# PaddlePaddle/MetaGym

Hardware: AMD Instinct MI355X
Metric: env-steps/sec (whole node) at 2^16 parallel envs; 1/2/4/8-GPU scaling (higher is better)
Workload: dtype f32/f64 mixed (reference choreography)

## Files before the change

### include/metagym_hip.h

```cpp
#ifndef METAGYM_HIP_H
#define METAGYM_HIP_H

#include <stddef.h>
#include <stdint.h>

#ifdef __cplusplus
extern "C" {
#endif

#define MG_ABI_VERSION 10

#define MG_OK 0
#define MG_ERR_NULL_POINTER (-1001)
#define MG_ERR_BAD_SIZE (-1002)
#define MG_ERR_BAD_CONFIG (-1003)
#define MG_ERR_UNSUPPORTED (-1004)

int mg_abi_version(void);
const char *mg_last_error(void);
const char *mg_target_arch(void);

int mg_selftest_philox(const uint32_t *ctr_key_d, uint32_t *out_d, int32_t n, void *stream);


// ... 63 lines not shown
                                const mg_quadrotor_state *state, const mg_quadrotor_autoreset *ar,
                                const float *action, float *obs, float *reward, double *reward64,
                                uint8_t *done, uint8_t *failed, void *stream);

typedef struct mg_quadrotor_plan { uint64_t opaque[128]; } mg_quadrotor_plan;

int mg_quadrotor_plan_init(mg_quadrotor_plan *plan, const mg_quadrotor_config *cfg,
                           const mg_quadrotor_autoreset *ar , int32_t n_envs,
                           const mg_quadrotor_state *state);
int mg_quadrotor_plan_step(const mg_quadrotor_plan *plan, int32_t n_steps, const float *action, float *obs,
                           float *reward, double *reward64, uint8_t *done, uint8_t *failed, void *stream);

typedef struct mg_quadrotor_fold {
    int32_t one_wave_form;
    uint32_t span;
    uint32_t base_v, base_w;
    uint32_t edge_v, edge_w;
    float pos_safe32;
    float fail_range_sq32;
    double fail_velocity, fail_w;
} mg_quadrotor_fold;

int mg_quadrotor_plan_fold(const mg_quadrotor_plan *plan, mg_quadrotor_fold *out);

typedef struct mg_quadrotor_tasks {
    const void *rows_d;
    const int32_t *task_id_d;
    const float *velocity_targets_d;
    int32_t n_tasks;
    int32_t all_simple;
    double dt;
} mg_quadrotor_tasks;

typedef struct mg_quadrotor_task_fold {
    float inertia_inv[9];
    float lm[4];
    float fail_range_sq32;
    float prec32;
    int32_t times;
    int32_t simple;
    double precision, half_dt2, dt;
    float init_velocity[3], init_angular_velocity[3];
    double init_velocity_noisy, init_angular_velocity_noisy;
} mg_quadrotor_task_fold;

int32_t mg_quadrotor_tasks_row_bytes(void);
// ... 599 lines not shown
```

### metagym_amd/_lib.py

```python
import ctypes as C
import os

from . import build as _build

ABI_VERSION = 10

MG_OK = 0


class MetaGymHipError(RuntimeError):
    pass


class QuadrotorConfig(C.Structure):
    _fields_ = [
        ("precision", C.c_double), ("quality", C.c_double),
        ("ct0", C.c_double), ("ct1", C.c_double), ("ct2", C.c_double),
        ("mm", C.c_double), ("jm", C.c_double), ("ra", C.c_double), ("phi", C.c_double),
        ("fail_velocity", C.c_double), ("fail_w", C.c_double), ("fail_range", C.c_double),
        ("min_voltage", C.c_double), ("max_voltage", C.c_double),
        ("dt", C.c_double), ("healthy_reward", C.c_double), ("z_offset", C.c_double),
        ("x_offset", C.c_int64), ("y_offset", C.c_int64),
        ("nt", C.c_int32), ("task", C.c_int32),
        ("inertia", C.c_float * 9), ("drag_m", C.c_float * 9), ("drag_f", C.c_float * 9),
# ... 267 lines not shown
                  "pyp", "pyv", "npp", "npv", "reward", "timec", "energy", "given", "st_d", "st_g", "st_a", "st_e", "st_w",
                  "rp_holder", "rp_priority"]
LIFTSIM_POLICY_ACTIONS, LIFTSIM_POLICY_RULE = 0, 1

_P = C.c_void_p
SIGNATURES = {
    "mg_abi_version": (C.c_int, []),
    "mg_last_error": (C.c_char_p, []),
    "mg_target_arch": (C.c_char_p, []),
    "mg_selftest_philox": (C.c_int, [_P, _P, C.c_int32, _P]),
    "mg_quadrotor_default_config": (C.c_int, [C.POINTER(QuadrotorConfig)]),
    "mg_quadrotor_velocity_targets": (C.c_int, [C.POINTER(QuadrotorConfig), C.c_int32, _P, _P, _P]),
    "mg_quadrotor_reset": (C.c_int, [C.POINTER(QuadrotorConfig), C.c_int32, C.POINTER(QuadrotorState),
                                     _P, _P, _P, _P, _P]),
    "mg_quadrotor_step": (C.c_int, [C.POINTER(QuadrotorConfig), C.c_int32, C.POINTER(QuadrotorState),
                                    _P, _P, _P, _P, _P, _P, _P]),
    "mg_quadrotor_step_autoreset": (C.c_int, [C.POINTER(QuadrotorConfig), C.c_int32, C.c_int32,
                                              C.POINTER(QuadrotorState), C.POINTER(QuadrotorAutoReset),
                                              _P, _P, _P, _P, _P, _P, _P]),
    "mg_quadrotor_plan_init": (C.c_int, [C.POINTER(QuadrotorPlan), C.POINTER(QuadrotorConfig),
                                         C.POINTER(QuadrotorAutoReset), C.c_int32, C.POINTER(QuadrotorState)]),
    "mg_quadrotor_plan_step": (C.c_int, [C.POINTER(QuadrotorPlan), C.c_int32, _P, _P, _P, _P, _P, _P, _P]),
    "mg_quadrotor_plan_fold": (C.c_int, [C.POINTER(QuadrotorPlan), C.POINTER(QuadrotorFold)]),
    "mg_quadrotor_tasks_row_bytes": (C.c_int32, []),
    "mg_quadrotor_tasks_fold": (C.c_int, [C.POINTER(QuadrotorConfig), C.POINTER(QuadrotorAutoReset), _P]),
    "mg_quadrotor_tasks_describe": (C.c_int, [_P, C.POINTER(QuadrotorTaskFold)]),
    "mg_quadrotor_tasks_step": (C.c_int, [C.POINTER(QuadrotorConfig), C.POINTER(QuadrotorTasks), C.c_int32, C.c_int32,
                                          C.POINTER(QuadrotorState), C.POINTER(QuadrotorAutoReset),
                                          _P, _P, _P, _P, _P, _P, _P]),
    "mg_quadrotor_tasks_reset": (C.c_int, [C.POINTER(QuadrotorConfig), C.POINTER(QuadrotorTasks), C.c_int32,
                                           C.POINTER(QuadrotorState), _P, _P, _P, _P, _P]),
    "mg_quadrotor_policy_param_count": (C.c_int32, [C.c_int32, C.c_int32]),
    "mg_quadrotor_policy_rollout": (C.c_int, [C.POINTER(QuadrotorConfig), C.POINTER(QuadrotorTasks), C.c_int32, C.c_int32,
                                              C.POINTER(QuadrotorState), C.POINTER(QuadrotorAutoReset),
                                              C.POINTER(QuadrotorPolicyDesc), _P, _P, _P, C.POINTER(QuadrotorPolicyRecords),
                                              C.POINTER(QuadrotorPolicyLast), _P]),
    "mg_quadrotor_rpolicy_param_count": (C.c_int32, [C.c_int32, C.c_int32]),
    "mg_quadrotor_rpolicy_rollout": (C.c_int, [C.POINTER(QuadrotorConfig), C.POINTER(QuadrotorTasks), C.c_int32, C.c_int32,
                                               C.POINTER(QuadrotorState), C.POINTER(QuadrotorAutoReset),
                                               C.POINTER(QuadrotorPolicyDesc), C.POINTER(QuadrotorRPolicyCarry), C.c_int32,
                                               _P, _P, _P, C.POINTER(QuadrotorPolicyRecords),
                                               C.POINTER(QuadrotorPolicyLast), _P]),
    "mg_quadrotor_rollout": (C.c_int, [C.POINTER(QuadrotorConfig), C.c_int32, C.c_int32,
                                       C.POINTER(QuadrotorState), _P, _P, _P, _P, _P, _P, _P]),
    "mg_maze_view_tables": (C.c_int, [C.c_int32, C.c_double, C.c_double, _P, _P]),
    "mg_maze_sample_tasks": (C.c_int, [C.POINTER(MazeSampleParams), C.c_int32, C.c_uint32, _P, _P, _P, _P, _P, _P,
# ... 132 lines not shown
```

### metagym_amd/csrc/quadrotor.hip

```cpp
#include <cstdlib>
#include <cstring>

#include "mg_common.h"
#include "mg_philox.h"

namespace {

#ifndef MG_QUAD_BLOCK
#define MG_QUAD_BLOCK 256
#endif
constexpr int BLOCK = MG_QUAD_BLOCK;
constexpr int WAVES_PER_BLOCK = BLOCK / mg::WAVE;
constexpr int OBS_DIM = 16;

struct QuadK {
    float phi32, phi_over_ra32, inv_jm32, mm32, prec32, ct0_32, ct1_32;
    float quality32, dt32, zoff32, healthy32, fail_range_sq32;
    float lm[4];
    float pc[12];
    float iinv[9];
    float df[9], dm[9];
    float cog[3];
    double prec, half_dt2, half_dt, ct2, quality, inv_quality;
    double min_v, max_v, fail_velocity, fail_w, healthy, xoff, yoff;
// ... 425 lines not shown
constexpr int AUX_PLAIN = 0, AUX_NT = 2, AUX_SC1 = 16, AUX_SC0_SC1 = 17, AUX_SC1_NT = 18;
constexpr bool st_policy_ok(int aux) {
    return aux == AUX_PLAIN || aux == AUX_NT || aux == AUX_SC1 || aux == AUX_SC0_SC1 || aux == AUX_SC1_NT;
}
constexpr bool ld_policy_ok(int aux) { return aux == AUX_PLAIN || aux == AUX_NT; }
#ifndef MG_QUAD_ST_STATE
#define MG_QUAD_ST_STATE 16
#endif
#ifndef MG_QUAD_ST_OBS
#define MG_QUAD_ST_OBS 16
#endif
#ifndef MG_QUAD_ST_SCALAR
#define MG_QUAD_ST_SCALAR 16
#endif
#ifndef MG_QUAD_STP_STATE
#define MG_QUAD_STP_STATE 2
#endif
#ifndef MG_QUAD_STP_OBS
#define MG_QUAD_STP_OBS 2
#endif
#ifndef MG_QUAD_STP_SCALAR
#define MG_QUAD_STP_SCALAR 2
#endif
#ifndef MG_QUAD_LD_STATE
#define MG_QUAD_LD_STATE 0
#endif
static_assert(st_policy_ok(MG_QUAD_ST_STATE) && st_policy_ok(MG_QUAD_ST_OBS) && st_policy_ok(MG_QUAD_ST_SCALAR) &&
              st_policy_ok(MG_QUAD_STP_STATE) && st_policy_ok(MG_QUAD_STP_OBS) && st_policy_ok(MG_QUAD_STP_SCALAR),
              "store policy: 0 plain, 2 nt, 16 sc1, 17 sc0 sc1, 18 sc1 nt");
static_assert(ld_policy_ok(MG_QUAD_LD_STATE), "load policy: 0 plain, 2 nt");
enum StoreClass { ST_STATE = 0, ST_OBS = 1, ST_SCALAR = 2 };
template <bool BUF, int CLS> constexpr int st_policy() {
    return CLS == ST_STATE ? (BUF ? MG_QUAD_ST_STATE : MG_QUAD_STP_STATE)
         : CLS == ST_OBS   ? (BUF ? MG_QUAD_ST_OBS : MG_QUAD_STP_OBS)
                           : (BUF ? MG_QUAD_ST_SCALAR : MG_QUAD_STP_SCALAR);
}
typedef float v4f __attribute__((ext_vector_type(4)));
typedef uint32_t v2u __attribute__((ext_vector_type(2)));
typedef uint32_t v4u __attribute__((ext_vector_type(4)));

__device__ __forceinline__ __amdgpu_buffer_rsrc_t rsrc_of(const void *base, uint32_t bytes) {
    return __builtin_amdgcn_make_buffer_rsrc(const_cast<void *>(base), (short)0, (int)bytes, 0x00020000);
}
template <typename T, int AUX = AUX_PLAIN> __device__ __forceinline__ T buf_ld(__amdgpu_buffer_rsrc_t r, uint32_t vo, uint32_t so) {
    static_assert(ld_policy_ok(AUX), "load policy");
    if constexpr (sizeof(T) == 4) return __builtin_bit_cast(T, __builtin_amdgcn_raw_buffer_load_b32(r, vo, so, AUX));
    else if constexpr (sizeof(T) == 8) return __builtin_bit_cast(T, __builtin_amdgcn_raw_buffer_load_b64(r, vo, so, AUX));
    else return __builtin_bit_cast(T, __builtin_amdgcn_raw_buffer_load_b128(r, vo, so, AUX));
}
template <int AUX, typename T> __device__ __forceinline__ void buf_st(T v, __amdgpu_buffer_rsrc_t r, uint32_t vo, uint32_t so) {
    static_assert(st_policy_ok(AUX), "store policy");
    if constexpr (sizeof(T) == 1) __builtin_amdgcn_raw_buffer_store_b8(__builtin_bit_cast(uint8_t, v), r, vo, so, AUX);
    else if constexpr (sizeof(T) == 4) __builtin_amdgcn_raw_buffer_store_b32(__builtin_bit_cast(uint32_t, v), r, vo, so, AUX);
    else if constexpr (sizeof(T) == 8) __builtin_amdgcn_raw_buffer_store_b64(__builtin_bit_cast(v2u, v), r, vo, so, AUX);
    else __builtin_amdgcn_raw_buffer_store_b128(__builtin_bit_cast(v4u, v), r, vo, so, AUX);
}
template <typename T> struct same_size_uint;
template <> struct same_size_uint<uint8_t> { typedef uint8_t type; };
// ... 3 lines not shown
template <> struct same_size_uint<double> { typedef uint64_t type; };
template <int AUX, typename T> __device__ __forceinline__ void st_stream(T *p, T v) {
    static_assert(st_policy_ok(AUX), "store policy");
    if constexpr (AUX == AUX_NT) __builtin_nontemporal_store(v, p);
    else if constexpr (AUX == AUX_PLAIN) *p = v;
    else if constexpr (AUX == AUX_SC1 && sizeof(T) <= 8) {
        typedef typename same_size_uint<T>::type U;
        __hip_atomic_store(reinterpret_cast<U *>(p), __builtin_bit_cast(U, v), __ATOMIC_RELAXED, __HIP_MEMORY_SCOPE_AGENT);
    } else {
        const uint64_t a = (uint64_t)p;
        const uint64_t base = ((uint64_t)(uint32_t)__builtin_amdgcn_readfirstlane((uint32_t)(a >> 32)) << 32) |
                              (uint64_t)(uint32_t)__builtin_amdgcn_readfirstlane((uint32_t)a);
        buf_st<AUX>(v, rsrc_of((const void *)base, mg::WAVE * OBS_DIM * 4), (uint32_t)(a - base), 0);
    }
}
template <bool BUF, int AUX = AUX_PLAIN, typename T> __device__ __forceinline__ T ld_soa(const T *a, int comps, int n, int c, int e) {
    if (!BUF) {
        if constexpr (AUX == AUX_NT) return __builtin_nontemporal_load(&a[(size_t)c * n + e]);
        else return a[(size_t)c * n + e];
    }
    return buf_ld<T, AUX>(rsrc_of(a, (uint32_t)comps * (uint32_t)n * sizeof(T)), (uint32_t)e * sizeof(T),
                          (uint32_t)c * (uint32_t)n * sizeof(T));
}
template <bool BUF, int CLS, typename T> __device__ __forceinline__ void st_soa(T *a, int comps, int n, int c, int e, T v) {
    if (!BUF) return st_stream<st_policy<false, CLS>()>(&a[(size_t)c * n + e], v);
    buf_st<st_policy<true, CLS>()>(v, rsrc_of(a, (uint32_t)comps * (uint32_t)n * sizeof(T)), (uint32_t)e * sizeof(T),
                                   (uint32_t)c * (uint32_t)n * sizeof(T));
}

template <bool ROT_FIRST = false, bool BUF = false>
__device__ __forceinline__ void load_state(const mg_quadrotor_state &st, int n, int e, Lane &s, int &ct) {
    if (ROT_FIRST) {
#pragma unroll
        for (int c = 0; c < 9; ++c) s.R[c] = ld_soa<BUF, MG_QUAD_LD_STATE>(st.rot, 9, n, c, e);
    }
    if (!ROT_FIRST) {
#pragma unroll
        for (int c = 0; c < 3; ++c) s.p[c] = ld_soa<BUF, MG_QUAD_LD_STATE>(st.pos, 3, n, c, e);
    }
#pragma unroll
    for (int c = 0; c < 3; ++c) s.v[c] = ld_soa<BUF, MG_QUAD_LD_STATE>(st.vel, 3, n, c, e);
#pragma unroll
    for (int c = 0; c < 3; ++c) s.w[c] = ld_soa<BUF, MG_QUAD_LD_STATE>(st.omega, 3, n, c, e);
    if (ROT_FIRST) {
#pragma unroll
        for (int c = 0; c < 3; ++c) s.p[c] = ld_soa<BUF, MG_QUAD_LD_STATE>(st.pos, 3, n, c, e);
    }
#pragma unroll
    for (int c = 0; c < 4; ++c) s.pw[c] = ld_soa<BUF, MG_QUAD_LD_STATE>(st.propw, 4, n, c, e);
    if (!ROT_FIRST) {
#pragma unroll
        for (int c = 0; c < 9; ++c) s.R[c] = ld_soa<BUF, MG_QUAD_LD_STATE>(st.rot, 9, n, c, e);
    }
    ct = ld_soa<BUF, MG_QUAD_LD_STATE>(st.ct, 1, n, 0, e);
}

__device__ __forceinline__ void derive_lane(Lane &s) {
    update_derived(s);
    s.power = 0.0f;
}

template <bool BUF = false>
__device__ __forceinline__ void load_lane(const mg_quadrotor_state &st, int n, int e, Lane &s, int &ct) {
    load_state<false, BUF>(st, n, e, s, ct);
    derive_lane(s);
}

template <bool BUF = false>
__device__ __forceinline__ void store_lane(const mg_quadrotor_state &st, int n, int e, const Lane &s, int ct) {
#pragma unroll
    for (int c = 0; c < 3; ++c) st_soa<BUF, ST_STATE>(st.pos, 3, n, c, e, s.p[c]);
#pragma unroll
    for (int c = 0; c < 3; ++c) st_soa<BUF, ST_STATE>(st.vel, 3, n, c, e, s.v[c]);
#pragma unroll
    for (int c = 0; c < 3; ++c) st_soa<BUF, ST_STATE>(st.omega, 3, n, c, e, s.w[c]);
#pragma unroll
    for (int c = 0; c < 4; ++c) st_soa<BUF, ST_STATE>(st.propw, 4, n, c, e, s.pw[c]);
#pragma unroll
    for (int c = 0; c < 9; ++c) st_soa<BUF, ST_STATE>(st.rot, 9, n, c, e, s.R[c]);
    st_soa<BUF, ST_STATE>(st.ct, 1, n, 0, e, ct);
}

template <bool BUF = false>
__device__ __forceinline__ void store_obs_wave(float *tile, const float *obs, float *out, int n, int e, int obs_dim) {
    if (!BUF && obs_dim != OBS_DIM) {
        if (e < n)
            for (int c = 0; c < obs_dim; ++c) out[(size_t)e * obs_dim + c] = obs[c];
        return;
    }
    const int lane = threadIdx.x & (mg::WAVE - 1);
    const int wave_base = e - lane;
    const bool full = (wave_base + mg::WAVE) <= n;
    if (full) {
#pragma unroll
        for (int c = 0; c < OBS_DIM; ++c) tile[lane * (OBS_DIM + 1) + c] = obs[c];
        __builtin_amdgcn_wave_barrier();
        float4 *dst = reinterpret_cast<float4 *>(out + (size_t)wave_base * OBS_DIM);
        const __amdgpu_buffer_rsrc_t r = rsrc_of(out, (uint32_t)n * (OBS_DIM * 4));
#pragma unroll
        for (int j = 0; j < 4; ++j) {
            const int q = j * mg::WAVE + lane;
            const int row = q >> 2, col = (q & 3) * 4;
            const float *src = &tile[row * (OBS_DIM + 1) + col];
            const v4f v{src[0], src[1], src[2], src[3]};
            if (BUF) buf_st<st_policy<true, ST_OBS>()>(v, r, (uint32_t)(wave_base * OBS_DIM + 4 * lane) * 4 + j * (mg::WAVE * 16), 0);
            else st_stream<st_policy<false, ST_OBS>()>(reinterpret_cast<v4f *>(dst + q), v);
        }
        __builtin_amdgcn_wave_barrier();
    } else if (e < n) {
        float4 *dst = reinterpret_cast<float4 *>(out + (size_t)e * OBS_DIM);
        const __amdgpu_buffer_rsrc_t r = rsrc_of(out, (uint32_t)n * (OBS_DIM * 4));
#pragma unroll
        for (int j = 0; j < 4; ++j) {
            const v4f v{obs[4 * j], obs[4 * j + 1], obs[4 * j + 2], obs[4 * j + 3]};
            if (BUF) buf_st<st_policy<true, ST_OBS>() & ~AUX_NT>(v, r, (uint32_t)e * (OBS_DIM * 4) + j * 16, 0);
            else if constexpr ((st_policy<false, ST_OBS>() & ~AUX_NT) == AUX_PLAIN) dst[j] = make_float4(v.x, v.y, v.z, v.w);
            else st_stream<st_policy<false, ST_OBS>() & ~AUX_NT>(reinterpret_cast<v4f *>(dst + j), v);
        }
    }
}

struct ResetDraw {
    double v[3], w[3], nv, nw;
};

__device__ __forceinline__ ResetDraw reset_draw(const QuadK &k, int e, uint32_t episode) {
    uint32_t r[8];
    const uint64_t gid = k.env_id_base + (uint64_t)e;
#pragma unroll
    for (int b = 0; b < 2; ++b)
        philox4x32_10((uint32_t)gid, (uint32_t)(gid >> 32), episode, (uint32_t)b, (uint32_t)k.seed,
                      (uint32_t)(k.seed >> 32), &r[4 * b]);
    const double inv32 = 1.0 / 4294967296.0;
    ResetDraw d;
#pragma unroll
    for (int c = 0; c < 3; ++c) {
        const double sv = ((r[6] >> c) & 1u) ? 1.0 : -1.0;
        const double sw = ((r[6] >> (3 + c)) & 1u) ? 1.0 : -1.0;
// ... 24 lines not shown
    s.nw = d.nw;
    s.power = 0.0f;
}


struct StepIO {
    const float *action;
    float *obs;
    float *reward;
    double *reward64;
    uint8_t *done;
    uint8_t *failed;
};

struct KArgs { QuadK k; mg_quadrotor_state st; StepIO io; int n; int n_steps; };
static_assert(sizeof(QuadK) == 448 && sizeof(KArgs) == 560, "kernel argument layout (the prologue touches its nine 64-byte lines)");
typedef const __attribute__((address_space(4))) KArgs KArgsC;
__device__ __forceinline__ KArgsC *kernargs_fresh() {
    KArgsC *p = (KArgsC *)__builtin_amdgcn_kernarg_segment_ptr();
    asm volatile("" : "+s"(p));
    return p;
}

enum StepForm { STEP_GENERIC = 0, STEP_STOCK = 1, STEP_STOCK_SHADOW = 2 };

#ifdef MG_QUAD_PHASE_STAMPS
constexpr int PHASE_STAMPS = 5, PHASE_SLOTS = 8, PHASE_MAX_WAVES = 4096;
__device__ uint64_t g_phase_stamps[PHASE_MAX_WAVES * PHASE_SLOTS];
#define MG_PHASE_STAMP(i)                                                                 \
    do {                                                                                  \
        if (SHADOW) {                                                                     \
            __builtin_amdgcn_sched_barrier(0);                                            \
            stamp[i] = __builtin_amdgcn_s_memrealtime();                                  \
            __builtin_amdgcn_sched_barrier(0);                                            \
        }                                                                                 \
    } while (0)
#else
#define MG_PHASE_STAMP(i) \
    do {                  \
    } while (0)
#endif
constexpr int STOCK_TIMES = 10;
#ifndef MG_QUAD_FASTPATH
#define MG_QUAD_FASTPATH 1
#endif
#ifndef MG_QUAD_SUBSTEP_UNROLL
#define MG_QUAD_SUBSTEP_UNROLL 9
#endif

template <bool SIMPLE, int FORM, bool XF = false, bool BUF = false, bool FLAT = false, bool HOVER = false>
__global__ __launch_bounds__(BLOCK) void quadrotor_step_kernel(QuadK k, mg_quadrotor_state st, StepIO io,
                                                               int n, int n_steps_arg) {
    constexpr bool STOCK = FORM != STEP_GENERIC;
    constexpr bool SHADOW = FORM == STEP_STOCK_SHADOW;
    static_assert(!STOCK || SIMPLE, "the stock forms are SIMPLE");
    static_assert(STOCK || !XF, "XF is an option of the stock forms");
    static_assert(SHADOW || !BUF, "BUF is an option of STEP_STOCK_SHADOW");
    static_assert(STOCK || !FLAT, "FLAT is an option of the stock forms");
    static_assert(SHADOW || !HOVER, "HOVER is an option of STEP_STOCK_SHADOW");
    constexpr bool FAST = SHADOW && MG_QUAD_FASTPATH;
    const int n_steps = SHADOW ? 1 : n_steps_arg;
    __shared__ float tiles[WAVES_PER_BLOCK][mg::WAVE * (OBS_DIM + 1)];
    const int e = blockIdx.x * BLOCK + threadIdx.x;
    const bool live = e < n;
    const int el = live ? e : n - 1;
    float *tile = tiles[threadIdx.x / mg::WAVE];

    {
        const uint32_t *ka = (const uint32_t *)__builtin_amdgcn_kernarg_segment_ptr();
        uint32_t touch = 0;
#pragma unroll
        for (int line = 0; line < (int)((sizeof(QuadK) + sizeof(mg_quadrotor_state) + sizeof(StepIO) + 8 + 63) / 64); ++line)
            touch |= ka[line * 16];
        asm volatile("" ::"s"(touch));
    }
#ifdef MG_QUAD_PHASE_STAMPS
    uint64_t stamp[PHASE_STAMPS];
    uint32_t fallbacks = 0;
    const uint64_t clock_in = __builtin_readcyclecounter();
#endif
    MG_PHASE_STAMP(0);
    bool ok = true;
    float4 a_next;
    Lane s;
    int ct;
    uint32_t episode = 0;
    ResetDraw rd;
    if (SHADOW) {
        episode = ld_soa<BUF>(st.episode, 1, n, 0, el);
        a_next = ld_soa<BUF>(reinterpret_cast<const float4 *>(io.action), 1, n, 0, el);
        load_state<true, BUF>(st, n, el, s, ct);
        __builtin_amdgcn_sched_barrier(0);
        rd = reset_draw(k, el, episode);
#pragma unroll
        for (int c = 0; c < 3; ++c) asm volatile("" : "+v"(rd.v[c]), "+v"(rd.w[c]));
        asm volatile("" : "+v"(rd.nv), "+v"(rd.nw));
        __builtin_amdgcn_sched_barrier(0);
        derive_lane(s);
        __builtin_amdgcn_sched_barrier(0);
    } else {
        a_next = reinterpret_cast<const float4 *>(io.action)[el];
        __builtin_amdgcn_sched_barrier(0);
        if (STOCK || k.auto_reset) episode = st.episode[el];
        load_lane(st, n, el, s, ct);
    }
    const uint32_t episode_in = episode;
    __builtin_amdgcn_s_waitcnt(0x0F70);
    MG_PHASE_STAMP(1);

    for (int t = 0; t < n_steps; ++t) {
        const size_t off = (size_t)t * n;
        const float4 a = a_next;
        if (t + 1 < n_steps)
            a_next = reinterpret_cast<const float4 *>(io.action)[off + n + el];
        const float av[4] = {a.x, a.y, a.z, a.w};
        float eff32[4];
#pragma unroll
        for (int i = 0; i < 4; ++i) {
            double d = (double)av[i];
            d = d > k.max_v ? k.max_v : (d < k.min_v ? k.min_v : d);
            eff32[i] = (float)d;
        }
// ... 33 lines not shown
                fail = 0;
#pragma unroll 1
                for (int it = 0; it < STOCK_TIMES; ++it) {
                    substep<SIMPLE, true, XF, false>(kf, s, eff32, it == STOCK_TIMES - 1, ok);
                    const int code = failure_code(kf, s);
                    fail = fail ? fail : code;
                }
#ifdef MG_QUAD_PHASE_STAMPS
                fallbacks += 1;
#endif
            }
        } else {
            for (int it = 0; it < k.times; ++it) {
                if (fail == 0) {
                    substep<SIMPLE>(k, s, eff32, it == k.times - 1, ok);
                    fail = failure_code(k, s);
                }
            }
        }
        MG_PHASE_STAMP(2);
        const KArgsC *kae = kernargs_fresh();
        const QuadK &ke = *(const QuadK *)&kae->k;
        const StepIO &ioe = *(const StepIO *)&kae->io;
        const bool vel_task = !SHADOW && ke.task == MG_QUADROTOR_TASK_VELOCITY_CONTROL;
        const bool hover_task = HOVER || ke.task == MG_QUADROTOR_TASK_HOVERING_CONTROL;
        const int tn_step = ct < ke.nt - 1 ? ct : ke.nt - 1;
        double reward = 0.0;
        int done = 1;
        if (fail == 0 && vel_task) {
            float bt[3];
            mv_f32(s.Ri, &ke.vtargets[3 * (ct - 1)], bt);
            double b_v[3];
            mv_f32f64(s.Ri, s.v, b_v);
            const double diff = (fabs((double)bt[0] - b_v[0]) + fabs((double)bt[1] - b_v[1])) + fabs((double)bt[2] - b_v[2]);
            const float energy = ke.dt32 * s.power;
            const double r = (ke.healthy32 < energy) ? -ke.healthy : -(double)energy;
            reward = r + (-0.001 * diff);
            done = 0;
            if (ct == ke.nt) { done = 1; ct = 0; }
        } else if (fail == 0) {
            const double new_pos[3] = {(double)s.p[0] + ke.xoff, (double)s.p[1] + ke.yoff,
                                       (double)(s.p[2] + ke.zoff32)};
            const bool hit = FLAT ? collision_flat(old_pos[2], new_pos[2]) : collision(ke, old_pos, new_pos);
            const float energy = ke.dt32 * s.power;
            double r = (ke.healthy32 < energy) ? -ke.healthy : -(double)energy;
            double task_reward = hit ? 0.0 : ke.healthy;
            if (hover_task) {
// ... 5 lines not shown
                    task_reward += (o > -20.0f) ? (double)o : -20.0;
                }
            }
            if (hover_task || ke.healthy32 < energy)
                reward = r + task_reward;
            else
                reward = (double)((float)r + (float)task_reward);
            done = 0;
            if (hit) { done = 1; ct = 0; }
            if (ct == ke.nt) { done = 1; ct = 0; }
        } else {
            ct = 0;
        }
        int tn = tn_step;
        if ((STOCK || ke.auto_reset) && done) {
            if (SHADOW) reset_apply(s, rd);
            else reset_apply(s, reset_draw(ke, el, episode));
            episode += 1;
            tn = ct < ke.nt - 1 ? ct : ke.nt - 1;
        }
        if (t + 1 < n_steps) asm volatile("" : "+v"(a_next.x), "+v"(a_next.y), "+v"(a_next.z), "+v"(a_next.w));
        if (t == n_steps - 1 && live) {
            const mg_quadrotor_state &ste = *(const mg_quadrotor_state *)&kae->st;
            store_lane<BUF>(ste, n, e, s, ct);
            if (episode != episode_in) st_soa<BUF, ST_STATE>(ste.episode, 1, n, 0, e, episode);
        }
        MG_PHASE_STAMP(3);
        __builtin_amdgcn_sched_barrier(0);
        float obs[OBS_DIM + 3];
        observe(ke, s, obs);
        if (vel_task) { obs[16] = ke.vtargets[3 * tn]; obs[17] = ke.vtargets[3 * tn + 1]; obs[18] = ke.vtargets[3 * tn + 2]; }
        store_obs_wave<BUF>(tile, obs, ioe.obs + off * ke.obs_dim, n, e, ke.obs_dim);
        MG_PHASE_STAMP(4);
        if (live) {
            if (BUF) {
                if (ioe.reward) st_soa<true, ST_SCALAR>(ioe.reward + off, 1, n, 0, e, (float)reward);
                if (ioe.reward64) st_soa<true, ST_SCALAR>(ioe.reward64 + off, 1, n, 0, e, reward);
                st_soa<true, ST_SCALAR>(ioe.done + off, 1, n, 0, e, (uint8_t)done);
                if (ioe.failed) st_soa<true, ST_SCALAR>(ioe.failed + off, 1, n, 0, e, (uint8_t)fail);
            } else {
                if (ioe.reward) st_stream<st_policy<false, ST_SCALAR>()>(&ioe.reward[off + e], (float)reward);
                if (ioe.reward64) st_stream<st_policy<false, ST_SCALAR>()>(&ioe.reward64[off + e], reward);
                st_stream<st_policy<false, ST_SCALAR>()>(&ioe.done[off + e], (uint8_t)done);
                if (ioe.failed) st_stream<st_policy<false, ST_SCALAR>()>(&ioe.failed[off + e], (uint8_t)fail);
            }
        }
    }
#ifdef MG_QUAD_PHASE_STAMPS
    if (SHADOW) {
        const uint32_t wave = (blockIdx.x * BLOCK + threadIdx.x) / mg::WAVE;
        if ((threadIdx.x & (mg::WAVE - 1)) == 0 && wave < PHASE_MAX_WAVES) {
            uint64_t *out = &g_phase_stamps[(size_t)wave * PHASE_SLOTS];
#pragma unroll
            for (int i = 0; i < PHASE_STAMPS; ++i) out[i] = stamp[i];
            out[5] = clock_in;
            out[6] = (uint64_t)__builtin_amdgcn_s_getreg((31 << 11) | 4) |
                     ((uint64_t)__builtin_amdgcn_s_getreg((31 << 11) | 20) << 32);
            out[7] = (uint64_t)fallbacks << 32;
        }
    }
#endif
}

__global__ __launch_bounds__(BLOCK) void quadrotor_reset_kernel(QuadK k, mg_quadrotor_state st,
                                                                const uint8_t *mask, const double *init_vel,
                                                                const double *init_omega, float *obs_out, int n) {
    const int e = blockIdx.x * BLOCK + threadIdx.x;
    if (e >= n) return;
    if (mask != nullptr && mask[e] == 0) return;
    Lane s;
#pragma unroll
    for (int c = 0; c < 3; ++c) {
// ... 168 lines not shown
    const float sx[4] = {1.0f, -1.0f, -1.0f, 1.0f}, sy[4] = {1.0f, 1.0f, -1.0f, -1.0f};
    if (!(c > 0.0f && c < INFINITY)) return false;
    for (int i = 0; i < 4; ++i)
        if (pc[3 * i] != sx[i] * c || pc[3 * i + 1] != sy[i] * c || pc[3 * i + 2] != 0.0f) return false;
    return true;
}

int check_state(const mg_quadrotor_state *s) {
    if (!s->pos || !s->vel || !s->omega || !s->propw || !s->rot || !s->ct)
        return mg::set_error(MG_ERR_NULL_POINTER, "mg_quadrotor_state has a NULL array");
    return MG_OK;
}

#ifdef MG_QUADROTOR_CORE_ONLY
}
#else
struct Plan {
    uint32_t magic;
    int32_t n, device, simple;
    int32_t stock;
    int32_t xframe;
    int32_t simds;
    int32_t lean;
    QuadK k;
    mg_quadrotor_state st;
};
constexpr uint32_t PLAN_MAGIC = 0x4d475150u;
static_assert(sizeof(Plan) <= sizeof(mg_quadrotor_plan), "mg_quadrotor_plan is too small for the folded constants");

int make_plan(Plan *p, const mg_quadrotor_config *cfg, const mg_quadrotor_autoreset *ar, int32_t n,
              const mg_quadrotor_state *state) {
    MG_REQUIRE_PTR(cfg);
    MG_REQUIRE_PTR(state);
    if (n <= 0) return mg::set_error(MG_ERR_BAD_SIZE, "n_envs=%d", n);
    if (int rc = check_state(state)) return rc;
    if (int rc = fold_config(cfg, &p->k)) return rc;
    if (ar != nullptr) {
        if (state->episode == nullptr)
            return mg::set_error(MG_ERR_NULL_POINTER, "fused auto-reset needs mg_quadrotor_state.episode");
        QuadK &k = p->k;
        k.auto_reset = 1;
        for (int i = 0; i < 3; ++i) { k.init_v_base[i] = ar->init_velocity[i]; k.init_w_base[i] = ar->init_angular_velocity[i]; }
        k.init_v_noisy = ar->init_velocity_noisy;
        k.init_w_noisy = ar->init_angular_velocity_noisy;
        k.seed = ar->seed;
        k.env_id_base = ar->env_id_base;
    }
    p->magic = PLAN_MAGIC;
    p->n = n;
    p->device = mg::device_of(state->pos);
    p->simple = (config_is_simple(cfg) && cfg->task != MG_QUADROTOR_TASK_VELOCITY_CONTROL) ? 1 : 0;
    const bool force_generic = getenv("MG_QUAD_GENERIC") != nullptr;
    p->stock = (!force_generic && p->simple && p->k.quality_recip_exact && p->k.times == STOCK_TIMES && p->k.auto_reset) ? 1 : 0;
    p->xframe = (p->stock && config_is_xframe(cfg)) ? 1 : 0;
    p->lean = (p->stock && fold_lean(&p->k) && (!p->xframe || p->k.lm[0] > 0.0f)) ? 1 : 0;
    p->simds = 0;
    int cus = 0;
    if (p->device >= 0 && hipDeviceGetAttribute(&cus, hipDeviceAttributeMultiprocessorCount, p->device) == hipSuccess)
        p->simds = 4 * cus;
    else
        (void)hipGetLastError();
    p->st = *state;
    return MG_OK;
}

typedef decltype(&quadrotor_step_kernel<false, STEP_GENERIC>) StepKernel;
template <bool... B>
StepKernel pick_shadow() { return quadrotor_step_kernel<true, STEP_STOCK_SHADOW, B...>; }
template <bool... B, typename... Rest>
StepKernel pick_shadow(bool b, Rest... rest) { return b ? pick_shadow<B..., true>(rest...) : pick_shadow<B..., false>(rest...); }

int launch_plan(const Plan *p, int32_t n_steps, const float *action, float *obs, float *reward, double *reward64,
                uint8_t *done, uint8_t *failed, void *stream) {
    MG_REQUIRE_PTR(action);
    MG_REQUIRE_PTR(obs);
    MG_REQUIRE_PTR(done);
    if (n_steps <= 0) return mg::set_error(MG_ERR_BAD_SIZE, "n_steps=%d", n_steps);
    mg::DeviceGuard guard(p->device);
    StepIO io{action, obs, reward, reward64, done, failed};
    const int n = p->n, grid = (n + BLOCK - 1) / BLOCK;
    const int waves = (n + mg::WAVE - 1) / mg::WAVE;
    const bool buf = (uint64_t)n * (OBS_DIM * sizeof(float)) < (1ull << 31);
    const bool flat = p->k.map == nullptr, hover = p->k.task == MG_QUADROTOR_TASK_HOVERING_CONTROL;
    StepKernel kern;
    if (p->stock && p->lean && n_steps == 1 && waves <= p->simds) {
        kern = pick_shadow(p->xframe != 0, buf, flat, hover);
    } else if (p->stock) {
        if (p->xframe) kern = flat ? quadrotor_step_kernel<true, STEP_STOCK, true, false, true> : quadrotor_step_kernel<true, STEP_STOCK, true>;
        else kern = flat ? quadrotor_step_kernel<true, STEP_STOCK, false, false, true> : quadrotor_step_kernel<true, STEP_STOCK>;
    } else if (p->simple) {
        kern = quadrotor_step_kernel<true, STEP_GENERIC>;
    } else {
        kern = quadrotor_step_kernel<false, STEP_GENERIC>;
    }
    hipLaunchKernelGGL(kern, dim3(grid), dim3(BLOCK), 0, (hipStream_t)stream, p->k, p->st, io, n, n_steps);
    return mg::check_launch("quadrotor_step_kernel");
}

int launch_steps(const mg_quadrotor_config *cfg, int32_t n, int32_t n_steps, const mg_quadrotor_state *state,
                 const float *action, float *obs, float *reward, double *reward64, uint8_t *done,
                 uint8_t *failed, void *stream, const mg_quadrotor_autoreset *ar = nullptr) {
    MG_REQUIRE_PTR(cfg);
    MG_REQUIRE_PTR(state);
    MG_REQUIRE_PTR(action);
    MG_REQUIRE_PTR(obs);
    MG_REQUIRE_PTR(done);
    Plan p;
    if (int rc = make_plan(&p, cfg, ar, n, state)) return rc;
    return launch_plan(&p, n_steps, action, obs, reward, reward64, done, failed, stream);
}
// ... 82 lines not shown
}

extern "C" int mg_quadrotor_plan_fold(const mg_quadrotor_plan *plan, mg_quadrotor_fold *out) {
    MG_REQUIRE_PTR(plan);
    MG_REQUIRE_PTR(out);
    const Plan *p = reinterpret_cast<const Plan *>(plan);
    if (p->magic != PLAN_MAGIC) return mg::set_error(MG_ERR_BAD_CONFIG, "mg_quadrotor_plan is not initialised");
    *out = mg_quadrotor_fold{};
    out->one_wave_form = !p->stock ? STEP_GENERIC : (p->lean ? STEP_STOCK_SHADOW : STEP_STOCK);
    out->span = LEAN_SPAN;
    out->fail_velocity = p->k.fail_velocity;
    out->fail_w = p->k.fail_w;
    out->fail_range_sq32 = p->k.fail_range_sq32;
    if (p->lean) {
        out->base_v = p->k.lean_base_v;
        out->base_w = p->k.lean_base_w;
        out->edge_v = p->k.lean_base_v + LEAN_SPAN;
        out->edge_w = p->k.lean_base_w + LEAN_SPAN;
        out->pos_safe32 = fold_pos_safe(p->k.fail_range_sq32);
    }
    return MG_OK;
}

#ifdef MG_QUAD_PHASE_STAMPS
extern "C" int mg_quadrotor_phase_stamps(uint64_t *host, int32_t max_waves) {
    MG_REQUIRE_PTR(host);
    const int32_t w = max_waves < PHASE_MAX_WAVES ? max_waves : PHASE_MAX_WAVES;
    if (hipMemcpyFromSymbol(host, HIP_SYMBOL(g_phase_stamps), (size_t)w * PHASE_SLOTS * sizeof(uint64_t)) != hipSuccess)
        return mg::set_error(MG_ERR_UNSUPPORTED, "hipMemcpyFromSymbol(g_phase_stamps) failed");
    return MG_OK;
}
#endif

extern "C" int mg_quadrotor_plan_step(const mg_quadrotor_plan *plan, int32_t n_steps, const float *action, float *obs,
                                      float *reward, double *reward64, uint8_t *done, uint8_t *failed, void *stream) {
    MG_REQUIRE_PTR(plan);
    const Plan *p = reinterpret_cast<const Plan *>(plan);
    if (p->magic != PLAN_MAGIC) return mg::set_error(MG_ERR_BAD_CONFIG, "mg_quadrotor_plan is not initialised");
    return launch_plan(p, n_steps, action, obs, reward, reward64, done, failed, stream);
}
#endif
```

### metagym_amd/quadrotor/env.py

```python
import ctypes as C
import json
import os
from collections.abc import Mapping

import numpy as np
import torch

from .. import _lib
from ..spaces import Box, Space

TASKS = {"no_collision": 0, "velocity_control": 1, "hovering_control": 2}

_raw_stream = getattr(torch._C, "_cuda_getCurrentRawStream", None) or (lambda index: torch.cuda.current_stream(index).cuda_stream)

DEFAULT_SIM_CONFIG = {
    "precision": 0.001, "quality": 0.5,
    "inertia": {"xx": 0.0135, "xy": 0.0, "xz": 0.0, "yy": 0.0135, "yz": 0.0, "zz": 0.024},
    "drag": {"m_xx": 0.074, "m_yy": 0.074, "m_zz": 0.0506, "f_xx": 0.12, "f_yy": 0.12, "f_zz": 0.10},
    "gravity_center": {"x": 0.0, "y": 0.0, "z": 0.0},
    "thrust": {"CT": ["1.538e-5", "-2.5e-4", "0.0"], "Mm": "0.010", "Jm": "2.573e-4", "RA": "0.2010",
               "phi": "0.017242179827506"},
    "propeller": [{"x": 0.18, "y": 0.18, "z": 0.0}, {"x": -0.18, "y": 0.18, "z": 0.0},
                  {"x": -0.18, "y": -0.18, "z": 0.0}, {"x": 0.18, "y": -0.18, "z": 0.0}],
    "fail": {"velocity": 100.0, "w": 1000.0, "range": 1000.0},
# ... 143 lines not shown
        self.auto_reset = bool(auto_reset)
        self._ar = _lib.QuadrotorAutoReset()
        cv = self.sim_config.get("init_velocity")
        cw = self.sim_config.get("init_angular_velocity") if cv is not None else None
        for i, ax in enumerate("xyz"):
            self._ar.init_velocity[i] = float(cv[ax]) if cv else 0.0
            self._ar.init_angular_velocity[i] = float(cw[ax]) if cw else 0.0
        self._ar.init_velocity_noisy = float(cv["noisy"]) if cv else 0.0
        self._ar.init_angular_velocity_noisy = float(cw["noisy"]) if cw else 0.0
        self._ar.seed = int(seed or 0) & 0xFFFFFFFFFFFFFFFF
        self._ar.env_id_base = int(env_id_base)
        self._plan = _lib.QuadrotorPlan()
        with torch.cuda.device(dev):
            rc = self._lib.mg_quadrotor_plan_init(self._plan, self._cfg, self._ar if self.auto_reset else None, N,
                                                  self._state)
        _lib.check(rc, "mg_quadrotor_plan_init")
        self._plan_ref = C.byref(self._plan)
        self._plan_step = self._lib.mg_quadrotor_plan_step
        self._dev_index = dev.index if dev.index is not None else torch.cuda.current_device()
        self._action_shape = (N, 4)
        self.task_table = None
        self.task_ids = None
        self._tasks = self._task_ids_host = self._tasks_keep = self.task_velocity_targets = None

    def reset(self, mask=None, seed=None, init_velocity=None, init_angular_velocity=None):
        N, dev = self.num_envs, self.device
        if seed is not None:
            self.np_random = np.random.RandomState(seed)
        if self.task_table is not None and (init_velocity is None or init_angular_velocity is None):
            u = self.np_random.random_sample((N, 4, 3))
            tb, ids = self.task_table, self._task_ids_host
            v = tb.init_velocity[ids] + (tb.init_velocity_noisy[ids][:, None] * u[:, 1]) * ((u[:, 0] > 0.5).astype(int) * 2 - 1.0)
            w = tb.init_angular_velocity[ids] + (tb.init_angular_velocity_noisy[ids][:, None] * u[:, 3]) * \
                ((u[:, 2] > 0.5).astype(int) * 2 - 1.0)
            init_velocity = v if init_velocity is None else init_velocity
            init_angular_velocity = w if init_angular_velocity is None else init_angular_velocity
        if init_velocity is None or init_angular_velocity is None:
            u = self.np_random.random_sample((N, 4, 3))
            cv, cw = self.sim_config.get("init_velocity"), self.sim_config.get("init_angular_velocity")
            v = np.zeros((N, 3))
            w = np.zeros((N, 3))
            if cv is not None:
                base = np.array([cv["x"], cv["y"], cv["z"]], dtype=np.float32)
                v = base + (float(cv["noisy"]) * u[:, 1]) * ((u[:, 0] > 0.5).astype(int) * 2 - 1.0)
            if cv is not None and cw is not None:
                base = np.array([cw["x"], cw["y"], cw["z"]], dtype=np.float32)
# ... 239 lines not shown
```

Baseline: 5.407 billion.

## Add lean multi-wave step form using buffer loads/stores for large env counts

Adds a STEP_STOCK_LEAN kernel form that reuses the single-step shadow fast path for env counts larger than one wave per SIMD. It loads action, episode and state through buffer loads and stores state, obs and scalars with a separate cache-policy set (default sc1). Previously such workloads fell back to the generic stock kernel. It also adds an MG_QUAD_FORM override and a query API exposing which form is chosen. The risk is that the single-step lean path and its store policies may not suit many-wave launches.

Measured after the change: 5.441 billion, median of 5. No clear change (+0.6%).

```diff
diff --git a/include/metagym_hip.h b/include/metagym_hip.h
--- a/include/metagym_hip.h
+++ b/include/metagym_hip.h
@@ -109,6 +109,8 @@
 } mg_quadrotor_fold;
 
 int mg_quadrotor_plan_fold(const mg_quadrotor_plan *plan, mg_quadrotor_fold *out);
+
+int mg_quadrotor_plan_form(const mg_quadrotor_plan *plan, int32_t n_steps, int32_t *form);
 
 typedef struct mg_quadrotor_tasks {
     const void *rows_d;
diff --git a/metagym_amd/_lib.py b/metagym_amd/_lib.py
--- a/metagym_amd/_lib.py
+++ b/metagym_amd/_lib.py
@@ -313,6 +313,7 @@
                                          C.POINTER(QuadrotorAutoReset), C.c_int32, C.POINTER(QuadrotorState)]),
     "mg_quadrotor_plan_step": (C.c_int, [C.POINTER(QuadrotorPlan), C.c_int32, _P, _P, _P, _P, _P, _P, _P]),
     "mg_quadrotor_plan_fold": (C.c_int, [C.POINTER(QuadrotorPlan), C.POINTER(QuadrotorFold)]),
+    "mg_quadrotor_plan_form": (C.c_int, [C.POINTER(QuadrotorPlan), C.c_int32, C.POINTER(C.c_int32)]),
     "mg_quadrotor_tasks_row_bytes": (C.c_int32, []),
     "mg_quadrotor_tasks_fold": (C.c_int, [C.POINTER(QuadrotorConfig), C.POINTER(QuadrotorAutoReset), _P]),
     "mg_quadrotor_tasks_describe": (C.c_int, [_P, C.POINTER(QuadrotorTaskFold)]),
diff --git a/metagym_amd/csrc/quadrotor.hip b/metagym_amd/csrc/quadrotor.hip
--- a/metagym_amd/csrc/quadrotor.hip
+++ b/metagym_amd/csrc/quadrotor.hip
@@ -471,18 +471,28 @@
 #ifndef MG_QUAD_STP_SCALAR
 #define MG_QUAD_STP_SCALAR 2
 #endif
+#ifndef MG_QUAD_STL_STATE
+#define MG_QUAD_STL_STATE 16
+#endif
+#ifndef MG_QUAD_STL_OBS
+#define MG_QUAD_STL_OBS 16
+#endif
+#ifndef MG_QUAD_STL_SCALAR
+#define MG_QUAD_STL_SCALAR 16
+#endif
 #ifndef MG_QUAD_LD_STATE
 #define MG_QUAD_LD_STATE 0
 #endif
 static_assert(st_policy_ok(MG_QUAD_ST_STATE) && st_policy_ok(MG_QUAD_ST_OBS) && st_policy_ok(MG_QUAD_ST_SCALAR) &&
-              st_policy_ok(MG_QUAD_STP_STATE) && st_policy_ok(MG_QUAD_STP_OBS) && st_policy_ok(MG_QUAD_STP_SCALAR),
+              st_policy_ok(MG_QUAD_STP_STATE) && st_policy_ok(MG_QUAD_STP_OBS) && st_policy_ok(MG_QUAD_STP_SCALAR) &&
+              st_policy_ok(MG_QUAD_STL_STATE) && st_policy_ok(MG_QUAD_STL_OBS) && st_policy_ok(MG_QUAD_STL_SCALAR),
               "store policy: 0 plain, 2 nt, 16 sc1, 17 sc0 sc1, 18 sc1 nt");
 static_assert(ld_policy_ok(MG_QUAD_LD_STATE), "load policy: 0 plain, 2 nt");
 enum StoreClass { ST_STATE = 0, ST_OBS = 1, ST_SCALAR = 2 };
-template <bool BUF, int CLS> constexpr int st_policy() {
-    return CLS == ST_STATE ? (BUF ? MG_QUAD_ST_STATE : MG_QUAD_STP_STATE)
-         : CLS == ST_OBS   ? (BUF ? MG_QUAD_ST_OBS : MG_QUAD_STP_OBS)
-                           : (BUF ? MG_QUAD_ST_SCALAR : MG_QUAD_STP_SCALAR);
+template <bool BUF, int CLS, bool MW = false> constexpr int st_policy() {
+    return CLS == ST_STATE ? (BUF ? (MW ? MG_QUAD_STL_STATE : MG_QUAD_ST_STATE) : MG_QUAD_STP_STATE)
+         : CLS == ST_OBS   ? (BUF ? (MW ? MG_QUAD_STL_OBS : MG_QUAD_ST_OBS) : MG_QUAD_STP_OBS)
+                           : (BUF ? (MW ? MG_QUAD_STL_SCALAR : MG_QUAD_ST_SCALAR) : MG_QUAD_STP_SCALAR);
 }
 typedef float v4f __attribute__((ext_vector_type(4)));
 typedef uint32_t v2u __attribute__((ext_vector_type(2)));
@@ -532,10 +542,10 @@
     return buf_ld<T, AUX>(rsrc_of(a, (uint32_t)comps * (uint32_t)n * sizeof(T)), (uint32_t)e * sizeof(T),
                           (uint32_t)c * (uint32_t)n * sizeof(T));
 }
-template <bool BUF, int CLS, typename T> __device__ __forceinline__ void st_soa(T *a, int comps, int n, int c, int e, T v) {
+template <bool BUF, int CLS, bool MW = false, typename T> __device__ __forceinline__ void st_soa(T *a, int comps, int n, int c, int e, T v) {
     if (!BUF) return st_stream<st_policy<false, CLS>()>(&a[(size_t)c * n + e], v);
-    buf_st<st_policy<true, CLS>()>(v, rsrc_of(a, (uint32_t)comps * (uint32_t)n * sizeof(T)), (uint32_t)e * sizeof(T),
-                                   (uint32_t)c * (uint32_t)n * sizeof(T));
+    buf_st<st_policy<true, CLS, MW>()>(v, rsrc_of(a, (uint32_t)comps * (uint32_t)n * sizeof(T)), (uint32_t)e * sizeof(T),
+                                       (uint32_t)c * (uint32_t)n * sizeof(T));
 }
 
 template <bool ROT_FIRST = false, bool BUF = false>
@@ -576,22 +586,22 @@
     derive_lane(s);
 }
 
-template <bool BUF = false>
+template <bool BUF = false, bool MW = false>
 __device__ __forceinline__ void store_lane(const mg_quadrotor_state &st, int n, int e, const Lane &s, int ct) {
 #pragma unroll
-    for (int c = 0; c < 3; ++c) st_soa<BUF, ST_STATE>(st.pos, 3, n, c, e, s.p[c]);
-#pragma unroll
-    for (int c = 0; c < 3; ++c) st_soa<BUF, ST_STATE>(st.vel, 3, n, c, e, s.v[c]);
-#pragma unroll
-    for (int c = 0; c < 3; ++c) st_soa<BUF, ST_STATE>(st.omega, 3, n, c, e, s.w[c]);
-#pragma unroll
-    for (int c = 0; c < 4; ++c) st_soa<BUF, ST_STATE>(st.propw, 4, n, c, e, s.pw[c]);
-#pragma unroll
-    for (int c = 0; c < 9; ++c) st_soa<BUF, ST_STATE>(st.rot, 9, n, c, e, s.R[c]);
-    st_soa<BUF, ST_STATE>(st.ct, 1, n, 0, e, ct);
-}
-
-template <bool BUF = false>
+    for (int c = 0; c < 3; ++c) st_soa<BUF, ST_STATE, MW>(st.pos, 3, n, c, e, s.p[c]);
+#pragma unroll
+    for (int c = 0; c < 3; ++c) st_soa<BUF, ST_STATE, MW>(st.vel, 3, n, c, e, s.v[c]);
+#pragma unroll
+    for (int c = 0; c < 3; ++c) st_soa<BUF, ST_STATE, MW>(st.omega, 3, n, c, e, s.w[c]);
+#pragma unroll
+    for (int c = 0; c < 4; ++c) st_soa<BUF, ST_STATE, MW>(st.propw, 4, n, c, e, s.pw[c]);
+#pragma unroll
+    for (int c = 0; c < 9; ++c) st_soa<BUF, ST_STATE, MW>(st.rot, 9, n, c, e, s.R[c]);
+    st_soa<BUF, ST_STATE, MW>(st.ct, 1, n, 0, e, ct);
+}
+
+template <bool BUF = false, bool MW = false>
 __device__ __forceinline__ void store_obs_wave(float *tile, const float *obs, float *out, int n, int e, int obs_dim) {
     if (!BUF && obs_dim != OBS_DIM) {
         if (e < n)
@@ -613,7 +623,7 @@
             const int row = q >> 2, col = (q & 3) * 4;
             const float *src = &tile[row * (OBS_DIM + 1) + col];
             const v4f v{src[0], src[1], src[2], src[3]};
-            if (BUF) buf_st<st_policy<true, ST_OBS>()>(v, r, (uint32_t)(wave_base * OBS_DIM + 4 * lane) * 4 + j * (mg::WAVE * 16), 0);
+            if (BUF) buf_st<st_policy<true, ST_OBS, MW>()>(v, r, (uint32_t)(wave_base * OBS_DIM + 4 * lane) * 4 + j * (mg::WAVE * 16), 0);
             else st_stream<st_policy<false, ST_OBS>()>(reinterpret_cast<v4f *>(dst + q), v);
         }
         __builtin_amdgcn_wave_barrier();
@@ -623,7 +633,7 @@
 #pragma unroll
         for (int j = 0; j < 4; ++j) {
             const v4f v{obs[4 * j], obs[4 * j + 1], obs[4 * j + 2], obs[4 * j + 3]};
-            if (BUF) buf_st<st_policy<true, ST_OBS>() & ~AUX_NT>(v, r, (uint32_t)e * (OBS_DIM * 4) + j * 16, 0);
+            if (BUF) buf_st<st_policy<true, ST_OBS, MW>() & ~AUX_NT>(v, r, (uint32_t)e * (OBS_DIM * 4) + j * 16, 0);
             else if constexpr ((st_policy<false, ST_OBS>() & ~AUX_NT) == AUX_PLAIN) dst[j] = make_float4(v.x, v.y, v.z, v.w);
             else st_stream<st_policy<false, ST_OBS>() & ~AUX_NT>(reinterpret_cast<v4f *>(dst + j), v);
         }
@@ -694,14 +704,14 @@
     return p;
 }
 
-enum StepForm { STEP_GENERIC = 0, STEP_STOCK = 1, STEP_STOCK_SHADOW = 2 };
+enum StepForm { STEP_GENERIC = 0, STEP_STOCK = 1, STEP_STOCK_SHADOW = 2, STEP_STOCK_LEAN = 3 };
 
 #ifdef MG_QUAD_PHASE_STAMPS
 constexpr int PHASE_STAMPS = 5, PHASE_SLOTS = 8, PHASE_MAX_WAVES = 4096;
 __device__ uint64_t g_phase_stamps[PHASE_MAX_WAVES * PHASE_SLOTS];
 #define MG_PHASE_STAMP(i)                                                                 \
     do {                                                                                  \
-        if (SHADOW) {                                                                     \
+        if (LEAN) {                                                                       \
             __builtin_amdgcn_sched_barrier(0);                                            \
             stamp[i] = __builtin_amdgcn_s_memrealtime();                                  \
             __builtin_amdgcn_sched_barrier(0);                                            \
@@ -725,13 +735,15 @@
                                                                int n, int n_steps_arg) {
     constexpr bool STOCK = FORM != STEP_GENERIC;
     constexpr bool SHADOW = FORM == STEP_STOCK_SHADOW;
+    constexpr bool LEAN = SHADOW || FORM == STEP_STOCK_LEAN;
+    constexpr bool MW = FORM == STEP_STOCK_LEAN;
     static_assert(!STOCK || SIMPLE, "the stock forms are SIMPLE");
     static_assert(STOCK || !XF, "XF is an option of the stock forms");
-    static_assert(SHADOW || !BUF, "BUF is an option of STEP_STOCK_SHADOW");
+    static_assert(LEAN || !BUF, "BUF is an option of the lean forms");
     static_assert(STOCK || !FLAT, "FLAT is an option of the stock forms");
-    static_assert(SHADOW || !HOVER, "HOVER is an option of STEP_STOCK_SHADOW");
-    constexpr bool FAST = SHADOW && MG_QUAD_FASTPATH;
-    const int n_steps = SHADOW ? 1 : n_steps_arg;
+    static_assert(LEAN || !HOVER, "HOVER is an option of the lean forms");
+    constexpr bool FAST = LEAN && MG_QUAD_FASTPATH;
+    const int n_steps = LEAN ? 1 : n_steps_arg;
     __shared__ float tiles[WAVES_PER_BLOCK][mg::WAVE * (OBS_DIM + 1)];
     const int e = blockIdx.x * BLOCK + threadIdx.x;
     const bool live = e < n;
@@ -770,6 +782,11 @@
         __builtin_amdgcn_sched_barrier(0);
         derive_lane(s);
         __builtin_amdgcn_sched_barrier(0);
+    } else if (MW) {
+        a_next = ld_soa<BUF>(reinterpret_cast<const float4 *>(io.action), 1, n, 0, el);
+        __builtin_amdgcn_sched_barrier(0);
+        episode = ld_soa<BUF>(st.episode, 1, n, 0, el);
+        load_lane<BUF>(st, n, el, s, ct);
     } else {
         a_next = reinterpret_cast<const float4 *>(io.action)[el];
         __builtin_amdgcn_sched_barrier(0);
@@ -849,7 +866,7 @@
         const KArgsC *kae = kernargs_fresh();
         const QuadK &ke = *(const QuadK *)&kae->k;
         const StepIO &ioe = *(const StepIO *)&kae->io;
-        const bool vel_task = !SHADOW && ke.task == MG_QUADROTOR_TASK_VELOCITY_CONTROL;
+        const bool vel_task = !LEAN && ke.task == MG_QUADROTOR_TASK_VELOCITY_CONTROL;
         const bool hover_task = HOVER || ke.task == MG_QUADROTOR_TASK_HOVERING_CONTROL;
         const int tn_step = ct < ke.nt - 1 ? ct : ke.nt - 1;
         double reward = 0.0;
@@ -901,22 +918,22 @@
         if (t + 1 < n_steps) asm volatile("" : "+v"(a_next.x), "+v"(a_next.y), "+v"(a_next.z), "+v"(a_next.w));
         if (t == n_steps - 1 && live) {
             const mg_quadrotor_state &ste = *(const mg_quadrotor_state *)&kae->st;
-            store_lane<BUF>(ste, n, e, s, ct);
-            if (episode != episode_in) st_soa<BUF, ST_STATE>(ste.episode, 1, n, 0, e, episode);
+            store_lane<BUF, MW>(ste, n, e, s, ct);
+            if (episode != episode_in) st_soa<BUF, ST_STATE, MW>(ste.episode, 1, n, 0, e, episode);
         }
         MG_PHASE_STAMP(3);
         __builtin_amdgcn_sched_barrier(0);
         float obs[OBS_DIM + 3];
         observe(ke, s, obs);
         if (vel_task) { obs[16] = ke.vtargets[3 * tn]; obs[17] = ke.vtargets[3 * tn + 1]; obs[18] = ke.vtargets[3 * tn + 2]; }
-        store_obs_wave<BUF>(tile, obs, ioe.obs + off * ke.obs_dim, n, e, ke.obs_dim);
+        store_obs_wave<BUF, MW>(tile, obs, ioe.obs + off * ke.obs_dim, n, e, ke.obs_dim);
         MG_PHASE_STAMP(4);
         if (live) {
             if (BUF) {
-                if (ioe.reward) st_soa<true, ST_SCALAR>(ioe.reward + off, 1, n, 0, e, (float)reward);
-                if (ioe.reward64) st_soa<true, ST_SCALAR>(ioe.reward64 + off, 1, n, 0, e, reward);
-                st_soa<true, ST_SCALAR>(ioe.done + off, 1, n, 0, e, (uint8_t)done);
-                if (ioe.failed) st_soa<true, ST_SCALAR>(ioe.failed + off, 1, n, 0, e, (uint8_t)fail);
+                if (ioe.reward) st_soa<true, ST_SCALAR, MW>(ioe.reward + off, 1, n, 0, e, (float)reward);
+                if (ioe.reward64) st_soa<true, ST_SCALAR, MW>(ioe.reward64 + off, 1, n, 0, e, reward);
+                st_soa<true, ST_SCALAR, MW>(ioe.done + off, 1, n, 0, e, (uint8_t)done);
+                if (ioe.failed) st_soa<true, ST_SCALAR, MW>(ioe.failed + off, 1, n, 0, e, (uint8_t)fail);
             } else {
                 if (ioe.reward) st_stream<st_policy<false, ST_SCALAR>()>(&ioe.reward[off + e], (float)reward);
                 if (ioe.reward64) st_stream<st_policy<false, ST_SCALAR>()>(&ioe.reward64[off + e], reward);
@@ -926,7 +943,7 @@
         }
     }
 #ifdef MG_QUAD_PHASE_STAMPS
-    if (SHADOW) {
+    if (LEAN) {
         const uint32_t wave = (blockIdx.x * BLOCK + threadIdx.x) / mg::WAVE;
         if ((threadIdx.x & (mg::WAVE - 1)) == 0 && wave < PHASE_MAX_WAVES) {
             uint64_t *out = &g_phase_stamps[(size_t)wave * PHASE_SLOTS];
@@ -1141,6 +1158,7 @@
     int32_t xframe;
     int32_t simds;
     int32_t lean;
+    int32_t forced;
     QuadK k;
     mg_quadrotor_state st;
 };
@@ -1169,7 +1187,14 @@
     p->n = n;
     p->device = mg::device_of(state->pos);
     p->simple = (config_is_simple(cfg) && cfg->task != MG_QUADROTOR_TASK_VELOCITY_CONTROL) ? 1 : 0;
-    const bool force_generic = getenv("MG_QUAD_GENERIC") != nullptr;
+    p->forced = -1;
+    if (const char *f = getenv("MG_QUAD_FORM")) {
+        static const char *const names[] = {"generic", "stock", "one_wave", "lean"};
+        for (int i = 0; i < 4; ++i)
+            if (strcmp(f, names[i]) == 0) p->forced = i;
+        if (p->forced < 0) return mg::set_error(MG_ERR_BAD_CONFIG, "MG_QUAD_FORM=%s (generic, stock, one_wave or lean)", f);
+    }
+    const bool force_generic = getenv("MG_QUAD_GENERIC") != nullptr || p->forced == STEP_GENERIC;
     p->stock = (!force_generic && p->simple && p->k.quality_recip_exact && p->k.times == STOCK_TIMES && p->k.auto_reset) ? 1 : 0;
     p->xframe = (p->stock && config_is_xframe(cfg)) ? 1 : 0;
     p->lean = (p->stock && fold_lean(&p->k) && (!p->xframe || p->k.lm[0] > 0.0f)) ? 1 : 0;
@@ -1184,10 +1209,18 @@
 }
 
 typedef decltype(&quadrotor_step_kernel<false, STEP_GENERIC>) StepKernel;
-template <bool... B>
-StepKernel pick_shadow() { return quadrotor_step_kernel<true, STEP_STOCK_SHADOW, B...>; }
-template <bool... B, typename... Rest>
-StepKernel pick_shadow(bool b, Rest... rest) { return b ? pick_shadow<B..., true>(rest...) : pick_shadow<B..., false>(rest...); }
+template <int FORM, bool... B>
+StepKernel pick_lean() { return quadrotor_step_kernel<true, FORM, B...>; }
+template <int FORM, bool... B, typename... Rest>
+StepKernel pick_lean(bool b, Rest... rest) { return b ? pick_lean<FORM, B..., true>(rest...) : pick_lean<FORM, B..., false>(rest...); }
+
+int plan_form(const Plan *p, int n_steps) {
+    if (!p->stock) return STEP_GENERIC;
+    if (!p->lean || n_steps != 1 || p->forced == STEP_STOCK) return STEP_STOCK;
+    if (p->forced == STEP_STOCK_SHADOW || p->forced == STEP_STOCK_LEAN) return p->forced;
+    const int waves = (p->n + mg::WAVE - 1) / mg::WAVE;
+    return waves <= p->simds ? STEP_STOCK_SHADOW : STEP_STOCK_LEAN;
+}
 
 int launch_plan(const Plan *p, int32_t n_steps, const float *action, float *obs, float *reward, double *reward64,
                 uint8_t *done, uint8_t *failed, void *stream) {
@@ -1198,13 +1231,15 @@
     mg::DeviceGuard guard(p->device);
     StepIO io{action, obs, reward, reward64, done, failed};
     const int n = p->n, grid = (n + BLOCK - 1) / BLOCK;
-    const int waves = (n + mg::WAVE - 1) / mg::WAVE;
     const bool buf = (uint64_t)n * (OBS_DIM * sizeof(float)) < (1ull << 31);
     const bool flat = p->k.map == nullptr, hover = p->k.task == MG_QUADROTOR_TASK_HOVERING_CONTROL;
     StepKernel kern;
-    if (p->stock && p->lean && n_steps == 1 && waves <= p->simds) {
-        kern = pick_shadow(p->xframe != 0, buf, flat, hover);
-    } else if (p->stock) {
+    const int form = plan_form(p, n_steps);
+    if (form == STEP_STOCK_SHADOW) {
+        kern = pick_lean<STEP_STOCK_SHADOW>(p->xframe != 0, buf, flat, hover);
+    } else if (form == STEP_STOCK_LEAN) {
+        kern = pick_lean<STEP_STOCK_LEAN>(p->xframe != 0, buf, flat, hover);
+    } else if (form == STEP_STOCK) {
         if (p->xframe) kern = flat ? quadrotor_step_kernel<true, STEP_STOCK, true, false, true> : quadrotor_step_kernel<true, STEP_STOCK, true>;
         else kern = flat ? quadrotor_step_kernel<true, STEP_STOCK, false, false, true> : quadrotor_step_kernel<true, STEP_STOCK>;
     } else if (p->simple) {
@@ -1333,6 +1368,16 @@
     return MG_OK;
 }
 
+extern "C" int mg_quadrotor_plan_form(const mg_quadrotor_plan *plan, int32_t n_steps, int32_t *form) {
+    MG_REQUIRE_PTR(plan);
+    MG_REQUIRE_PTR(form);
+    const Plan *p = reinterpret_cast<const Plan *>(plan);
+    if (p->magic != PLAN_MAGIC) return mg::set_error(MG_ERR_BAD_CONFIG, "mg_quadrotor_plan is not initialised");
+    if (n_steps <= 0) return mg::set_error(MG_ERR_BAD_SIZE, "n_steps=%d", n_steps);
+    *form = plan_form(p, n_steps);
+    return MG_OK;
+}
+
 #ifdef MG_QUAD_PHASE_STAMPS
 extern "C" int mg_quadrotor_phase_stamps(uint64_t *host, int32_t max_waves) {
     MG_REQUIRE_PTR(host);
diff --git a/metagym_amd/quadrotor/env.py b/metagym_amd/quadrotor/env.py
--- a/metagym_amd/quadrotor/env.py
+++ b/metagym_amd/quadrotor/env.py
@@ -189,6 +189,13 @@
         self.task_table = None
         self.task_ids = None
         self._tasks = self._task_ids_host = self._tasks_keep = self.task_velocity_targets = None
+
+    STEP_FORMS = ("generic", "stock", "one_wave", "lean")
+
+    def step_form(self, n_steps=1):
+        form = C.c_int32(-1)
+        _lib.check(self._lib.mg_quadrotor_plan_form(self._plan, int(n_steps), C.byref(form)), "mg_quadrotor_plan_form")
+        return self.STEP_FORMS[form.value]
 
     def reset(self, mask=None, seed=None, init_velocity=None, init_angular_velocity=None):
         N, dev = self.num_envs, self.device
```
